# cptq/SignNet-BasisNet

Hardware: AMD Instinct MI355X
Metric: graphs/sec SignNet+GINE forward, ZINC batch=128 k=16 (higher is better)
Workload: dtype f32

## Files before the change

### signnet_basisnet_amd/csrc/fused_common.hpp

```cpp
#pragma once
#include "common.hpp"

namespace sn {

#ifdef SN_PROFILE
static __device__ long long g_prof[64];
#define SN_STAMP(i) do { if (sn_prof_on && blockIdx.x == 0 && threadIdx.x == 0) g_prof[i] = clock64(); } while (0)
#define SN_ACCUM(i, t0) do { if (sn_prof_on && blockIdx.x == 0 && threadIdx.x == 0) g_prof[i] += clock64() - (t0); } while (0)
#define SN_PROF_ON(cond) const bool sn_prof_on = (cond)
#else
#define SN_STAMP(i) do { } while (0)
#define SN_ACCUM(i, t0) do { } while (0)
#define SN_PROF_ON(cond) do { } while (0)
#endif

__device__ __forceinline__ f32x4 ld4(const float* __restrict__ p) {
  float4 t = *reinterpret_cast<const float4*>(p);
  return f32x4{t.x, t.y, t.z, t.w};
}
__device__ __forceinline__ f32x4 lds_ld4(const float* p) {
  float4 t = *reinterpret_cast<const float4*>(p);
  return f32x4{t.x, t.y, t.z, t.w};
}
__device__ __forceinline__ void lds_st4(float* p, f32x4 v) {
// ... 36 lines not shown
}
__device__ __forceinline__ Split8 split8(f32x4 a, f32x4 b) {
  const float x[8] = {a[0], a[1], a[2], a[3], b[0], b[1], b[2], b[3]};
  float h[8], m[8], l[8];
#pragma unroll
  for (int i = 0; i < 8; ++i) {
    h[i] = __uint_as_float(__float_as_uint(x[i]) & 0xffff0000u);
    const float r = x[i] - h[i];
    m[i] = __uint_as_float(__float_as_uint(r) & 0xffff0000u);
    l[i] = r - m[i];
  }
  Split8 s;
#pragma unroll
  for (int i = 0; i < 4; ++i) {
    s.h[i] = pack_hi16(h[2 * i], h[2 * i + 1]);
    s.m[i] = pack_hi16(m[2 * i], m[2 * i + 1]);
    s.l[i] = pack_hi16(l[2 * i], l[2 * i + 1]);
  }
  return s;
}
__device__ __forceinline__ void split4(f32x4 a, Split8& s, int half) {
  float h[4], m[4], l[4];
#pragma unroll
  for (int i = 0; i < 4; ++i) {
    h[i] = __uint_as_float(__float_as_uint(a[i]) & 0xffff0000u);
    const float r = a[i] - h[i];
    m[i] = __uint_as_float(__float_as_uint(r) & 0xffff0000u);
    l[i] = r - m[i];
  }
#pragma unroll
  for (int i = 0; i < 2; ++i) {
    s.h[2 * half + i] = pack_hi16(h[2 * i], h[2 * i + 1]);
    s.m[2 * half + i] = pack_hi16(m[2 * i], m[2 * i + 1]);
    s.l[2 * half + i] = pack_hi16(l[2 * i], l[2 * i + 1]);
  }
}
template <int NT>
__device__ __forceinline__ void split_rows(const f32x4 (&in)[NT], Split8 (&xs)[(NT + 1) / 2]) {
#pragma unroll
  for (int kb = 0; kb < (NT + 1) / 2; ++kb)
    xs[kb] = split8(in[2 * kb], (2 * kb + 1 < NT) ? in[2 * kb + 1] : f32x4{0.f, 0.f, 0.f, 0.f});
}
__device__ __forceinline__ f32x4 mfma_bf(u32x4 a, u32x4 b, f32x4 c) {
  return __builtin_amdgcn_mfma_f32_16x16x32_bf16(__builtin_bit_cast(bf16x8, a), __builtin_bit_cast(bf16x8, b), c, 0, 0, 0);
}
template <int N>
__device__ __forceinline__ void wait_vmcnt() { asm volatile("s_waitcnt vmcnt(%0)" ::"n"(N) : "memory"); }
__device__ __forceinline__ void lds_barrier() {
  asm volatile("s_waitcnt lgkmcnt(0)" ::: "memory");
  __builtin_amdgcn_s_barrier();
  asm volatile("" ::: "memory");
}

template <int NT, int NW = 4, int RING = SPLIT_RING>
struct WRing {
  static constexpr int NKB = (NT + 1) / 2;
  static constexpr int NF = 3 * NKB;
  static constexpr int NFE = NF + SPLIT_EPI;
  static constexpr int CHUNK = NFE * 1024;
  static constexpr int BYTES = RING * CHUNK;
  static constexpr int DEPTH = RING;
  static constexpr int LPC = (NFE + NW - 1) / NW;
  lds_char_t* base;
  int pos;
  int wave, lane;

  __device__ __forceinline__ void init(void* lds_base, int wave_, int lane_) {
    base = (lds_char_t*)lds_base; pos = 0; wave = wave_; lane = lane_;
  }
  template <int N>
  __device__ __forceinline__ void wait_shares() const { wait_vmcnt<N * LPC>(); }
  __device__ __forceinline__ int slot_of(int c) const {
    const int x = pos + c;
    if (RING == 3) return x - 3 * ((x * 43) >> 7);
    if (RING == 4) return x & 3;
    return x % RING;
  }
  __device__ __forceinline__ void issue(const void* w, int c, int slot) const {
    const __amdgpu_buffer_rsrc_t rs = weight_rsrc(reinterpret_cast<const float*>(w), 0x7fffffff);
    int wo = wave * 1024;
    asm volatile("" : "+s"(wo));
    lds_char_t* dst = base + slot * CHUNK + wo;
    const int src = c * CHUNK + wo;
#pragma unroll
    for (int f = 0; f < LPC; ++f) {
      int fo = NW * 1024 * f;
      if (NW * f + NW - 1 >= NFE) {
        const int last = (NFE - 1) * 1024 - wo;
        fo = fo < last ? fo : last;
      }
      __builtin_amdgcn_raw_ptr_buffer_load_lds(rs, (lds_void_t*)(dst + fo), 16, lane * 16, src + fo, 0, 0);
    }
  }
  __device__ __forceinline__ void prologue(const void* w, int nchunks) {
    lds_barrier();
    pos = 0;
#pragma unroll
    for (int c = 0; c < RING; ++c)
      if (c < nchunks) issue(w, c, c);
    if (nchunks >= RING) wait_shares<RING - 1>(); else wait_vmcnt<0>();
    lds_barrier();
  }
  __device__ __forceinline__ void drain() const { wait_vmcnt<0>(); }
};

struct WFrag { u32x4 h, m, l; };

template <int PREC>
__device__ __forceinline__ WFrag read_wfrag(const lds_char_t* p) {
  typedef __attribute__((address_space(3))) const u32x4 lds_u32x4;
  WFrag f;
  f.h = *(lds_u32x4*)(p);
  if constexpr (PREC <= PREC_HIGH) f.m = *(lds_u32x4*)(p + 1024); else f.m = u32x4{0u, 0u, 0u, 0u};
  if constexpr (PREC == PREC_HIGHEST) f.l = *(lds_u32x4*)(p + 2048); else f.l = u32x4{0u, 0u, 0u, 0u};
  return f;
}
template <int PREC, bool SWAP>
__device__ __forceinline__ void mm_reduced(const WFrag& f, const Split8& x, int kb, f32x4& a0, f32x4& a1) {
  static_assert(PREC == PREC_HIGH || PREC == PREC_MEDIUM, "the six-product form is written out at its call sites");
  if constexpr (PREC == PREC_HIGH) {
    a1 = SWAP ? mfma_bf(x.h, f.m, a1) : mfma_bf(f.m, x.h, a1);
    a0 = SWAP ? mfma_bf(x.m, f.h, a0) : mfma_bf(f.h, x.m, a0);
    a0 = SWAP ? mfma_bf(x.h, f.h, a0) : mfma_bf(f.h, x.h, a0);
  } else {
    f32x4& a = (kb & 1) ? a1 : a0;
    a = SWAP ? mfma_bf(x.h, f.h, a) : mfma_bf(f.h, x.h, a);
  }
}

template <int NT, int NTO, bool SWAP, bool EPIV = true, int NW = 4, int RING = SPLIT_RING, int PREC = PREC_HIGHEST, typename Pre, typename Epi>
__device__ __forceinline__ void wg_gemm_split(WRing<NT, NW, RING>& ring, const void* w, const void* wnext, bool live,
                                              const Split8 (&xs)[(NT + 1) / 2], Pre pre, Epi epi) {
  using R = WRing<NT, NW, RING>;
  constexpr int NKB = R::NKB;
  constexpr bool CHAIN = NTO >= RING;
  if (!CHAIN) ring.prologue(w, NTO);
  typedef __attribute__((address_space(3))) const f32x4 lds_f32x4;
  int sl[RING];
#pragma unroll
  for (int i = 0; i < RING; ++i) sl[i] = ring.slot_of(i);
  auto slot = [&](int c) { return sl[c % RING]; };
  auto stage = [&](int ot) {
    if (CHAIN) {
      const int pc = ot + RING;
      if (pc < NTO) ring.issue(w, pc, slot(ot)); else ring.issue(wnext, pc - NTO, slot(ot));
    }
  };
  if (live) {
    int ln16 = ring.lane * 16;
    asm volatile("" : "+v"(ln16));
    const lds_char_t* lbase = ring.base + ln16;
    auto rd = [&](int c, int kb) { return read_wfrag<PREC>(lbase + slot(c) * R::CHUNK + kb * 3072); };
    auto mm = [&](const WFrag& f, const Split8& x, int kb, f32x4& a0, f32x4& a1) {
      if constexpr (PREC != PREC_HIGHEST) {
        mm_reduced<PREC, SWAP>(f, x, kb, a0, a1);
      } else if (!SWAP) {
        a1 = mfma_bf(f.l, x.h, a1);
        a0 = mfma_bf(f.m, x.h, a0);
        a1 = mfma_bf(f.h, x.l, a1);
        a0 = mfma_bf(f.h, x.m, a0);
        a1 = mfma_bf(f.m, x.m, a1);
        a0 = mfma_bf(f.h, x.h, a0);
      } else {
        a1 = mfma_bf(x.h, f.l, a1);
        a0 = mfma_bf(x.h, f.m, a0);
        a1 = mfma_bf(x.l, f.h, a1);
        a0 = mfma_bf(x.m, f.h, a0);
        a1 = mfma_bf(x.m, f.m, a1);
        a0 = mfma_bf(x.h, f.h, a0);
      }
    };
    WFrag fa = rd(0, 0), fb;
#pragma unroll
    for (int ot = 0; ot < NTO; ++ot) {
      f32x4 a0 = {0.f, 0.f, 0.f, 0.f}, a1 = {0.f, 0.f, 0.f, 0.f};
      f32x4 e0 = {0.f, 0.f, 0.f, 0.f}, e1 = e0, e2 = e0;
      if (EPIV) {
        const lds_char_t* pe = lbase + slot(ot) * R::CHUNK + R::NF * 1024;
        e0 = *(lds_f32x4*)(pe); e1 = *(lds_f32x4*)(pe + 1024); e2 = *(lds_f32x4*)(pe + 2048);
      }
      const f32x4 pv = pre(ot);
#pragma unroll
      for (int kb = 0; kb + 1 < NKB; ++kb) {
        fb = rd(ot, kb + 1);
        __builtin_amdgcn_sched_barrier(0);
        mm(fa, xs[kb], kb, a0, a1);
        __builtin_amdgcn_sched_barrier(0);
        fa = fb;
      }
      if (CHAIN) {
        asm volatile("s_waitcnt lgkmcnt(0)" ::: "memory");
        ring.template wait_shares<RING - 2>();
        __builtin_amdgcn_s_barrier();
        asm volatile("" ::: "memory");
        stage(ot);
      }
      if (ot + 1 < NTO) fb = rd(ot + 1, 0);
      __builtin_amdgcn_sched_barrier(0);
      mm(fa, xs[NKB - 1], NKB - 1, a0, a1);
      __builtin_amdgcn_sched_barrier(0);
      epi(ot, a0 + a1, e0, e1, e2, pv);
      fa = fb;
    }
  } else if (CHAIN) {
#pragma unroll
    for (int ot = 0; ot < NTO; ++ot) {
      ring.template wait_shares<RING - 2>();
      __builtin_amdgcn_s_barrier();
      asm volatile("" ::: "memory");
      stage(ot);
    }
  }
  ring.pos = ring.slot_of(NTO);
}

constexpr int LAG_RING = 4;

template <int NT, int NW>
__device__ __forceinline__ void ring_prologue3(WRing<NT, NW, LAG_RING>& ring, const void* w) {
  lds_barrier();
  ring.pos = 0;
  ring.issue(w, 0, 0);
  ring.issue(w, 1, 1);
  ring.issue(w, 2, 2);
  ring.template wait_shares<2>();
  lds_barrier();
}

template <int NT, int NW>
__device__ __forceinline__ void ring_prologue3_issue(WRing<NT, NW, LAG_RING>& ring, const void* w) {
  lds_barrier();
  ring.pos = 0;
  ring.issue(w, 0, 0);
  ring.issue(w, 1, 1);
  ring.issue(w, 2, 2);
}

template <int NT, int NTO, int BAR_KB, int NW, int PREC = PREC_HIGHEST, typename Pre, typename Epi>
__device__ __forceinline__ void wg_gemm_split_lag(WRing<NT, NW, LAG_RING>& ring, const void* w, const void* wnext, bool live,
                                                  const Split8 (&xs)[(NT + 1) / 2], Pre pre, Epi epi) {
  using R = WRing<NT, NW, LAG_RING>;
  constexpr int NKB = R::NKB;
  static_assert(NTO >= 3 && BAR_KB >= 0 && BAR_KB < NKB, "look-ahead of three chunks; the barrier sits in front of a K block of the tile");
  typedef __attribute__((address_space(3))) const f32x4 lds_f32x4;
  int sl[LAG_RING];
#pragma unroll
  for (int i = 0; i < LAG_RING; ++i) sl[i] = ring.slot_of(i);
  auto slot = [&](int c) { return sl[c % LAG_RING]; };
  auto sync_stage = [&](int ot) {
    ring.template wait_shares<1>();
    __builtin_amdgcn_s_barrier();
    asm volatile("" ::: "memory");
    const int pc = ot + 3;
    if (pc < NTO) ring.issue(w, pc, slot(pc)); else ring.issue(wnext, pc - NTO, slot(pc));
  };
  if (live) {
    int ln16 = ring.lane * 16;
    asm volatile("" : "+v"(ln16));
    const lds_char_t* lbase = ring.base + ln16;
    auto rd = [&](int c, int kb) { return read_wfrag<PREC>(lbase + slot(c) * R::CHUNK + kb * 3072); };
    WFrag fa = rd(0, 0), fb;
#pragma unroll
    for (int ot = 0; ot < NTO; ++ot) {
      f32x4 a0 = {0.f, 0.f, 0.f, 0.f}, a1 = {0.f, 0.f, 0.f, 0.f};
      const lds_char_t* pe = lbase + slot(ot) * R::CHUNK + R::NF * 1024;
      const f32x4 e0 = *(lds_f32x4*)(pe), e1 = *(lds_f32x4*)(pe + 1024), e2 = *(lds_f32x4*)(pe + 2048);
      const f32x4 pv = pre(ot);
#pragma unroll
      for (int kb = 0; kb < NKB; ++kb) {
        if (kb == BAR_KB) sync_stage(ot);
        if (kb + 1 < NKB) fb = rd(ot, kb + 1);
        else if (ot + 1 < NTO) fb = rd(ot + 1, 0);
        __builtin_amdgcn_sched_barrier(0);
        if constexpr (PREC != PREC_HIGHEST) {
          mm_reduced<PREC, false>(fa, xs[kb], kb, a0, a1);
        } else {
          a1 = mfma_bf(fa.l, xs[kb].h, a1);
          a0 = mfma_bf(fa.m, xs[kb].h, a0);
          a1 = mfma_bf(fa.h, xs[kb].l, a1);
          a0 = mfma_bf(fa.h, xs[kb].m, a0);
          a1 = mfma_bf(fa.m, xs[kb].m, a1);
          a0 = mfma_bf(fa.h, xs[kb].h, a0);
        }
        __builtin_amdgcn_sched_barrier(0);
        fa = fb;
      }
      epi(ot, a0 + a1, e0, e1, e2, pv);
    }
  } else {
#pragma unroll
    for (int ot = 0; ot < NTO; ++ot) sync_stage(ot);
  }
  ring.pos = ring.slot_of(NTO);
}

__device__ __forceinline__ float row_allsum(float v) {
  v += __shfl_xor(v, 16, 64);
  v += __shfl_xor(v, 32, 64);
  return v;
}

struct NoPre { __device__ __forceinline__ f32x4 operator()(int) const { return f32x4{0.f, 0.f, 0.f, 0.f}; } };

}
```

### signnet_basisnet_amd/csrc/fused_rho.hip

```cpp
#include "fused_common.hpp"

namespace sn {

constexpr int RHO_R = SN_RHO_BIN_ROWS;

struct RhoStruct {
  const float* x;
  const float* eigvals;
  const int32_t* graph_ptr;
  const int32_t* rho_bin0;
  const int32_t* meta;
  int B;
  int kmax;
  int K;
  float* out_sum;
  const int32_t* node_graph;
  int N;
  const int32_t* bin_mem;
};

template <int NT, bool HP = false>
__device__ __forceinline__ void masked_layernorm(f32x4 (&v)[NT], const float* gamma , const float* beta ,
                                                 float eps, int d, int g, bool valid) {
  float s = 0.f;
#pragma unroll
  for (int kk = 0; kk < NT; ++kk) s += (v[kk][0] + v[kk][1]) + (v[kk][2] + v[kk][3]);
  const float mean = row_allsum(s) / (float)d;
  const bool last_ok = 16 * (NT - 1) + 4 * g < d;
  float q = 0.f;
#pragma unroll
  for (int kk = 0; kk < NT; ++kk) {
#pragma unroll
    for (int t = 0; t < 4; ++t) {
      const bool real = HP ? (16 * kk + 4 * g < d) : (kk + 1 < NT || last_ok);
      const float dlt = real ? v[kk][t] - mean : 0.f;
      q += dlt * dlt;
    }
  }
  const float rstd = 1.0f / sqrtf(row_allsum(q) / (float)d + eps);
#pragma unroll
  for (int kk = 0; kk < NT; ++kk) {
    const int c = 16 * kk + 4 * g;
    const f32x4 ga = lds_ld4(gamma + c), be = lds_ld4(beta + c);
    f32x4 o;
#pragma unroll
    for (int t = 0; t < 4; ++t) o[t] = valid ? (v[kk][t] - mean) * rstd * ga[t] + be[t] : 0.f;
    v[kk] = o;
  }
}

__device__ __forceinline__ float group_allmax(float v) {
  v = fmaxf(v, __shfl_xor(v, 16, 64));
  return fmaxf(v, __shfl_xor(v, 32, 64));
}
__device__ __forceinline__ float dpp_add(float v, int ctrl_sel) {
  const int x = __float_as_int(v);
  int y;
  switch (ctrl_sel) {
    case 0: y = __builtin_amdgcn_update_dpp(0, x, 0xB1, 0xf, 0xf, true); break;
    case 1: y = __builtin_amdgcn_update_dpp(0, x, 0x4E, 0xf, 0xf, true); break;
    case 2: y = __builtin_amdgcn_update_dpp(0, x, 0x141, 0xf, 0xf, true); break;
    default: y = __builtin_amdgcn_update_dpp(0, x, 0x140, 0xf, 0xf, true); break;
  }
  return v + __int_as_float(y);
}
__device__ __forceinline__ float tile_rowsum(float v) {
  v = dpp_add(v, 0);
  v = dpp_add(v, 1);
  v = dpp_add(v, 2);
  return dpp_add(v, 3);
}

template <int NT, bool REGATTN, bool ONE, bool HP = false, int NW = 4, int PREC = PREC_HIGHEST, bool RES3 = false>
__global__ __launch_bounds__(64 * NW, REGATTN ? (RES3 ? 3 : 2) : 1) void k_rho_fused(RhoStruct S, sn_rho_params P) {
  static_assert(NW == 4 || (NW == 8 && REGATTN), "eight waves: the register-attention variants only (no 64-row LDS images)");
  static_assert(!RES3 || (REGATTN && ONE && NW == 4), "three resident workgroups: the one-layer register-attention form only");
  constexpr int NTHR = 64 * NW;
  constexpr int D = 16 * NT;
  constexpr int LD = D + 4;
  constexpr int DKMAX = (D + 3) / 4;
  constexpr int NKB = (NT + 1) / 2;
  using Ring = WRing<NT, NW>;
  extern __shared__ __align__(1024) unsigned char lds_raw[];
  float* A = reinterpret_cast<float*>(lds_raw + Ring::BYTES);
  float* Bm = A + RHO_R * LD;
  __shared__ int s_graph;
  const int lane = threadIdx.x & 63, wave = __builtin_amdgcn_readfirstlane(threadIdx.x >> 6);
  const int r = wave * 16 + (lane & 15), g = lane >> 4, li = lane & 15;
  const int nbins = REGATTN ? (S.N + NW - 1) / NW : S.meta[4];
  const int d = P.d, H = P.heads, dk = d / H;
  f32x4 x[NT];
  int pf_gs = 0, pf_n = 0;
  auto fetch_rows = [&](int node_) {
    int slot_ = lane & 15, g_ = g;
    asm volatile("" : "+v"(slot_), "+v"(g_));
    const bool ok = node_ < S.N && slot_ < S.K;
    const float* xr = S.x + (ok ? ((int64_t)node_ * S.K + slot_) : (int64_t)0) * d;
#pragma unroll
    for (int kk = 0; kk < NT; ++kk) {
      const int c = 16 * kk + 4 * g_;
      const bool inb = HP ? c < d : (kk + 1 < NT || c < d);
      x[kk] = ld4(xr + (inb ? c : 0));
    }
  };
  auto fetch_graph = [&](int node_) {
    const int32_t* p = S.node_graph + (node_ < S.N ? node_ : 0);
    int gi;
    asm volatile("s_load_dword %0, %1, 0x0\n\ts_waitcnt lgkmcnt(0)" : "=s"(gi) : "s"(p) : "memory");
    const int32_t* q = S.graph_ptr + gi;
    long long rng;
    asm volatile("s_load_dwordx2 %0, %1, 0x0\n\ts_waitcnt lgkmcnt(0)" : "=s"(rng) : "s"(q) : "memory");
    pf_gs = (int)(rng & 0xffffffffll);
    pf_n = (int)(rng >> 32) - pf_gs;
  };
#ifdef SN_RHO_OLDSTART
  constexpr bool EARLY = false;
#else
  constexpr bool EARLY = REGATTN && (ONE || NT < 8);
#endif
  const int err = S.meta[5];
  const float temp = sqrtf((float)dk);
  const float rtemp = 1.0f / temp;
  { SN_PROF_ON(true); SN_STAMP(13); }
  float* lnv = reinterpret_cast<float*>(lds_raw + Ring::BYTES) + (REGATTN ? 0 : 2 * RHO_R * LD);
  Ring ring;
  ring.init(lds_raw, wave, lane);
  const void* wfirst = P.n_layers > 0 ? P.layers[0].wq : nullptr;
  const bool stream = NT >= SPLIT_RING && wfirst != nullptr && nbins > (int)blockIdx.x;
  if constexpr (EARLY && ONE && NT >= SPLIT_RING) {
    if (nbins <= (int)blockIdx.x) return;
    const int node0 = __builtin_amdgcn_readfirstlane((int)blockIdx.x * NW + wave);
    fetch_rows(node0);
    static_assert(4 * (D / 4) <= NTHR, "one float4 per thread covers the four vectors");
    const int li4 = (int)threadIdx.x < 4 * (D / 4) ? (int)threadIdx.x : 0;
    const sn_rho_layer& L0 = P.layers[0];
    const float *p0 = L0.ln1_g, *p1 = L0.ln1_b, *p2 = L0.ln2_g, *p3 = L0.ln2_b;
    asm volatile("" : "+s"(p0), "+s"(p1), "+s"(p2), "+s"(p3));
    const int lv = li4 / (D / 4), lc = 4 * (li4 - lv * (D / 4));
    typedef __attribute__((address_space(1))) const float gfloat_t;
    gfloat_t* src = (gfloat_t*)(lv == 0 ? p0 : (lv == 1 ? p1 : (lv == 2 ? p2 : p3)));
    const f32x4 lnr = f32x4{src[lc], src[lc + 1], src[lc + 2], src[lc + 3]};
    ring.pos = 0;
#pragma unroll
    for (int c = 0; c < Ring::DEPTH; ++c) ring.issue(wfirst, c, c);
    fetch_graph(node0);
    {
      typedef __attribute__((address_space(3))) float lds_float_t;
      const unsigned la = (unsigned)(size_t)(lds_float_t*)(lnv + 4 * li4);
      asm volatile("ds_write_b128 %0, %1" :: "v"(la), "v"(lnr) : "memory");
    }
    ring.template wait_shares<Ring::DEPTH - 1>();
    lds_barrier();
    if (err != 0) { ring.drain(); return; }
  } else {
    if constexpr (EARLY) {
      if (nbins > (int)blockIdx.x) {
        const int node0 = __builtin_amdgcn_readfirstlane((int)blockIdx.x * NW + wave);
        fetch_rows(node0);
        fetch_graph(node0);
      }
    } else {
      if (err != 0) return;
    }
    for (int i = threadIdx.x; i < P.n_layers * 4 * D; i += NTHR) {
      const int l = i / (4 * D), v = (i / D) & 3, c = i % D;
      const sn_rho_layer& Lq = P.layers[l];
      const float* src = v == 0 ? Lq.ln1_g : (v == 1 ? Lq.ln1_b : (v == 2 ? Lq.ln2_g : Lq.ln2_b));
      lnv[i] = src[c];
    }
    __syncthreads();
    if (stream) ring.prologue(wfirst, NT);
    if constexpr (EARLY) {
      if (err != 0) { ring.drain(); return; }
    }
  }

  for (int bin = blockIdx.x; bin < nbins; bin += gridDim.x) {
    SN_PROF_ON(bin == (int)blockIdx.x);
    SN_STAMP(0);
    int gs, n, kg, q, slot, node, kv, u0;
    bool unit_ok;
    if constexpr (REGATTN) {
      q = wave;
      slot = lane & 15;
      node = __builtin_amdgcn_readfirstlane(bin * NW + wave);
      unit_ok = node < S.N;
      if constexpr (EARLY) {
        gs = pf_gs;
        n = pf_n;
      } else {
        const int gi = unit_ok ? S.node_graph[node] : 0;
        gs = S.graph_ptr[gi];
        n = S.graph_ptr[gi + 1] - gs;
      }
      kg = (S.kmax > 0 && n > S.kmax) ? S.kmax : n;
      kv = unit_ok ? kg : 0;
      u0 = q * 16;
    } else {
      __syncthreads();
      for (int gq = threadIdx.x; gq < S.B; gq += NTHR)
        if (S.rho_bin0[gq] <= bin && bin < S.rho_bin0[gq + 1]) s_graph = gq;
      __syncthreads();
      const int gi = s_graph;
      gs = S.graph_ptr[gi];
      n = S.graph_ptr[gi + 1] - gs;
      kg = (S.kmax > 0 && n > S.kmax) ? S.kmax : n;
      const int pad = ((kg + 15) >> 4) << 4;
      const int upb = RHO_R / pad;
      q = r / pad;
      slot = r - q * pad;
      const int u = (bin - S.rho_bin0[gi]) * upb + q;
      unit_ok = q < upb && u < n;
      node = gs + u;
      kv = unit_ok ? kg : 0;
      u0 = q * pad;
    }
    const bool valid = unit_ok && slot < kg;
    constexpr bool mfma_attn = REGATTN;
    const bool wave_live = RES3 || __ballot(valid) != 0ull;
    float* Ar = A + r * LD;
    float* Br = Bm + r * LD;
// ... 144 lines not shown
            const float pj = expf(s - m);
            z += pj;
#pragma unroll
            for (int c = 0; c < DKMAX; c += 4)
              if (c < dk) { const f32x4 v4 = lds_ld4(vr + c); oh[c] += pj * v4[0]; oh[c + 1] += pj * v4[1]; oh[c + 2] += pj * v4[2]; oh[c + 3] += pj * v4[3]; }
          }
        } else {
          for (int j = 0; j < kv; ++j) {
            const float* kr = Bm + (u0 + j) * LD + hc;
            float s = 0.f;
#pragma unroll
            for (int c = 0; c < DKMAX; ++c)
              if (c < dk) s += qh[c] * kr[c];
            m = fmaxf(m, s);
          }
          for (int j = 0; j < kv; ++j) {
            const float* kr = Bm + (u0 + j) * LD + hc;
            const float* vr = A + (u0 + j) * LD + hc;
            float s = 0.f;
#pragma unroll
            for (int c = 0; c < DKMAX; ++c)
              if (c < dk) s += qh[c] * kr[c];
            const float pj = expf(s - m);
            z += pj;
#pragma unroll
            for (int c = 0; c < DKMAX; ++c)
              if (c < dk) oh[c] += pj * vr[c];
          }
        }
        const float zi = (kv > 0) ? 1.0f / z : 0.f;
        lds_barrier();
#pragma unroll
        for (int c = 0; c < DKMAX; ++c)
          if (c < dk) Br[hc + c] = oh[c] * zi;
        if (H * dk < D) {
          for (int c = H * dk + g; c < D; c += 4) Br[c] = 0.f;
        }
#pragma unroll
        for (int kk = 0; kk < NT; ++kk) o[kk] = lds_ld4(Br + 16 * kk + 4 * g);
        }
      }
      SN_STAMP(5);
      if (wave_live) split_rows<NT>(o, sp);
      if (ONE) load_x();
      wg_gemm_split<NT, NT, false, false, NW, SPLIT_RING, PREC>(ring, Lp.wfc, Lp.w1, wave_live, sp, NoPre(), [&](int ot, f32x4 acc, f32x4, f32x4, f32x4, f32x4) { x[ot] = acc + x[ot]; });
      SN_STAMP(6);
      if (wave_live) {
        int gl = g;
        asm volatile("" : "+v"(gl));
        masked_layernorm<NT, HP>(x, lnv + (l * 4 + 0) * D, lnv + (l * 4 + 1) * D, P.ln_eps, d, gl, valid);
        split_rows<NT>(x, sp);
      }
      SN_STAMP(7);
      wg_gemm_split<NT, NT, false, true, NW, SPLIT_RING, PREC>(ring, Lp.w1, Lp.w2, wave_live, sp, NoPre(), [&](int ot, f32x4 acc, f32x4 b1, f32x4, f32x4, f32x4) { o[ot] = relu4(acc + b1); });
      SN_STAMP(8);
      if (wave_live) split_rows<NT>(o, sp);
#ifdef SN_PROFILE
      asm volatile("" :: "v"(sp[0].h), "v"(last_plane<PREC>(sp[NKB - 1])));
#endif
      SN_STAMP(14);
      wg_gemm_split<NT, NT, false, true, NW, SPLIT_RING, PREC>(ring, Lp.w2, wafter, wave_live, sp, NoPre(), [&](int ot, f32x4 acc, f32x4 b2, f32x4, f32x4, f32x4) { x[ot] = acc + b2 + x[ot]; });
      SN_STAMP(9);
      if (wave_live) {
        int gl = g;
        asm volatile("" : "+v"(gl));
        masked_layernorm<NT, HP>(x, lnv + (l * 4 + 2) * D, lnv + (l * 4 + 3) * D, P.ln_eps, d, gl, valid);
      }
      SN_STAMP(10);
    }
    if (mfma_attn) {
      if (wave_live) {
        float* orow = S.out_sum + (int64_t)node * d;
        int g_ = g;
        asm volatile("" : "+v"(g_));
#pragma unroll
        for (int kk = 0; kk < NT; ++kk) {
          f32x4 s;
#pragma unroll
          for (int t = 0; t < 4; ++t) s[t] = tile_rowsum(valid ? x[kk][t] : 0.f);
          const int c = 16 * kk + 4 * g_;
          if (li == 0 && unit_ok && (HP ? c < d : (kk + 1 < NT || c < d))) *reinterpret_cast<float4*>(orow + c) = make_float4(s[0], s[1], s[2], s[3]);
        }
      }
      if (EARLY && bin + (int)gridDim.x < nbins) {
        const int nnode = __builtin_amdgcn_readfirstlane((bin + (int)gridDim.x) * NW + wave);
        fetch_rows(nnode);
        fetch_graph(nnode);
      }
    } else {
#pragma unroll
      for (int kk = 0; kk < NT; ++kk) lds_st4(Br + 16 * kk + 4 * g, valid ? x[kk] : f32x4{0.f, 0.f, 0.f, 0.f});
      __syncthreads();
      if (valid && slot == 0) {
        float* orow = S.out_sum + (int64_t)node * d;
#pragma unroll
        for (int kk = 0; kk < NT; ++kk) {
          const int c = 16 * kk + 4 * g;
          f32x4 s = {0.f, 0.f, 0.f, 0.f};
          for (int j = 0; j < kv; ++j) s += lds_ld4(Bm + (u0 + j) * LD + c);
          if (kk + 1 < NT || c < d) *reinterpret_cast<float4*>(orow + c) = make_float4(s[0], s[1], s[2], s[3]);
        }
      }
    }
  }
  { SN_PROF_ON(true); SN_STAMP(11); }
  ring.drain();
}

template <int NT, bool ONE, bool COLS, int PREC = PREC_HIGHEST>
__global__ __launch_bounds__(RHO_R * 4, ONE ? 2 : 1) void k_rho_wide(RhoStruct S, sn_rho_params P) {
  static_assert(NT == 4 || NT == 8, "head width 16 or 32");
  constexpr int D = 16 * NT;
  constexpr int LD = D + 4;
  constexpr int NKB = (NT + 1) / 2;
  constexpr int CPH = NT / 4;
  using Ring = WRing<NT>;
  extern __shared__ __align__(1024) unsigned char lds_raw[];
  float* IMG = reinterpret_cast<float*>(lds_raw + Ring::BYTES);
  float* lnv = IMG + RHO_R * LD;
  const int lane = threadIdx.x & 63, wave = __builtin_amdgcn_readfirstlane(threadIdx.x >> 6);
  const int r = wave * 16 + (lane & 15), g = lane >> 4, li = lane & 15;
  const int nb_raw = COLS ? S.meta[7] : S.meta[4];
  const int m_err = S.meta[5] | (COLS ? S.meta[1] : 0);
  const int nbins = m_err != 0 ? 0 : nb_raw;
  const int d = P.d;
  const float rtemp = 1.0f / sqrtf((float)(d / P.heads));
  Ring ring;
  ring.init(lds_raw, wave, lane);
  const void* wfirst = P.n_layers > 0 ? P.layers[0].wq : nullptr;
  if constexpr (ONE) {
    static_assert(4 * (D / 4) <= RHO_R * 4, "one float4 per thread covers the four vectors");
    const int li4 = (int)threadIdx.x < 4 * (D / 4) ? (int)threadIdx.x : 0;
    const sn_rho_layer& L0 = P.layers[0];
    const float *p0 = L0.ln1_g, *p1 = L0.ln1_b, *p2 = L0.ln2_g, *p3 = L0.ln2_b;
    asm volatile("" : "+s"(p0), "+s"(p1), "+s"(p2), "+s"(p3));
    const int lv = li4 / (D / 4), lc = 4 * (li4 - lv * (D / 4));
    typedef __attribute__((address_space(1))) const float gfloat_t;
    gfloat_t* src = (gfloat_t*)(lv == 0 ? p0 : (lv == 1 ? p1 : (lv == 2 ? p2 : p3)));
    const f32x4 lnr = f32x4{src[lc], src[lc + 1], src[lc + 2], src[lc + 3]};
    if (nbins <= (int)blockIdx.x) return;
    ring.pos = 0;
#pragma unroll
    for (int c = 0; c < Ring::DEPTH; ++c) ring.issue(wfirst, c, c);
    {
      typedef __attribute__((address_space(3))) float lds_float_t;
      const unsigned la = (unsigned)(size_t)(lds_float_t*)(lnv + 4 * li4);
      asm volatile("ds_write_b128 %0, %1" :: "v"(la), "v"(lnr) : "memory");
    }
    ring.template wait_shares<Ring::DEPTH - 1>();
    lds_barrier();
  } else {
    for (int i = threadIdx.x; i < P.n_layers * 4 * D; i += RHO_R * 4) {
      const int l = i / (4 * D), v = (i / D) & 3, c = i % D;
      const sn_rho_layer& Lq = P.layers[l];
      const float* src = v == 0 ? Lq.ln1_g : (v == 1 ? Lq.ln1_b : (v == 2 ? Lq.ln2_g : Lq.ln2_b));
      lnv[i] = src[c];
    }
    __syncthreads();
    if (wfirst != nullptr && nbins > (int)blockIdx.x) ring.prologue(wfirst, NT);
  }
  float* IMGr = IMG + r * LD;

  for (int bin = blockIdx.x; bin < nbins; bin += gridDim.x) {
    int m_off[8], m_len[8], m_node[8], m_gs[8];
    if constexpr (COLS) {
      typedef int i32x16 __attribute__((ext_vector_type(16)));
      i32x16 rw;
      {
        const int32_t* rec = S.bin_mem + (int64_t)bin * 16;
        asm volatile("s_load_dwordx16 %0, %1, 0x0\n\ts_waitcnt lgkmcnt(0)" : "=s"(rw) : "s"(rec) : "memory");
      }
#pragma unroll
      for (int k = 0; k < 8; ++k) {
        const int w0 = rw[2 * k], g0 = rw[2 * k + 1];
        const int n = ((w0 >> 25) & 63) + 1;
        m_off[k] = (w0 >> 19) & 63;
        m_len[k] = (w0 >= 0 && n <= S.K) ? n : 0;
        m_node[k] = g0 + ((w0 >> 13) & 63);
        m_gs[k] = g0;
      }
    } else {
      int lo = 0, hi = S.B;
      while (hi - lo > 1) {
        const int mid = (lo + hi) >> 1;
        if (S.rho_bin0[mid] <= bin) lo = mid; else hi = mid;
      }
      const int gs = S.graph_ptr[lo], n = S.graph_ptr[lo + 1] - gs;
      const int kg = (S.kmax > 0 && n > S.kmax) ? S.kmax : n;
      const int pad = ((kg + 15) >> 4) << 4;
      const int upb = RHO_R / pad;
      const int ub = (bin - S.rho_bin0[lo]) * upb;
#pragma unroll
      for (int k = 0; k < 8; ++k) {
        m_off[k] = k * pad;
        m_len[k] = (k < upb && ub + k < n) ? kg : 0;
        m_node[k] = gs + ub + k;
        m_gs[k] = gs;
      }
    }
    int u0 = 0, kv = 0, node = 0, gsr = 0;
    int klo = RHO_R, khi = 0;
#pragma unroll
    for (int k = 0; k < 8; ++k) {
      if (r >= m_off[k] && r < m_off[k] + m_len[k]) { u0 = m_off[k]; kv = m_len[k]; node = m_node[k]; gsr = m_gs[k]; }
      if (m_len[k] > 0 && m_off[k] < wave * 16 + 16 && m_off[k] + m_len[k] > wave * 16) {
        klo = min(klo, m_off[k]);
        khi = max(khi, m_off[k] + m_len[k]);
      }
    }
// ... 58 lines not shown
#pragma unroll
          for (int h = 0; h < 4; ++h) {
            float m = -INFINITY;
#pragma unroll
            for (int kt = 0; kt < 4; ++kt)
#pragma unroll
              for (int t = 0; t < 4; ++t)
                if ((unsigned)(16 * kt + 4 * g + t - u0) < (unsigned)kv) m = fmaxf(m, sc[h][kt][t]);
            m = group_allmax(m);
            float z = 0.f;
#pragma unroll
            for (int kt = 0; kt < 4; ++kt)
#pragma unroll
              for (int t = 0; t < 4; ++t) {
                const float e = ((unsigned)(16 * kt + 4 * g + t - u0) < (unsigned)kv) ? expf(sc[h][kt][t] - m) : 0.f;
                sc[h][kt][t] = e;
                z += e;
              }
            z = row_allsum(z);
            const float zi = (kv > 0 && z > 0.f) ? 1.0f / z : 0.f;
#pragma unroll
            for (int kt = 0; kt < 4; ++kt)
#pragma unroll
              for (int t = 0; t < 4; ++t) sc[h][kt][t] *= zi;
          }
        }
        lds_barrier();
        wg_gemm_split<NT, NT, false, false, 4, SPLIT_RING, PREC>(ring, Lp.wv, Lp.wfc, wave_live, sp, NoPre(), [&](int ot, f32x4 acc, f32x4, f32x4, f32x4, f32x4) { lds_st4(IMGr + 16 * ot + 4 * g, acc); });
        lds_barrier();
#pragma unroll
        for (int ot = 0; ot < NT; ++ot) {
          f32x4 acc = {0.f, 0.f, 0.f, 0.f};
#pragma unroll
          for (int kt = 0; kt < 4; ++kt)
            if (wave_live && kt >= kt_lo && kt < kt_hi) {
              const float* vr = IMG + (16 * kt + 4 * g) * LD + 16 * ot + li;
              acc = mfma16(vr[0], sc[ot / CPH][kt][0], acc);
              acc = mfma16(vr[LD], sc[ot / CPH][kt][1], acc);
              acc = mfma16(vr[2 * LD], sc[ot / CPH][kt][2], acc);
              acc = mfma16(vr[3 * LD], sc[ot / CPH][kt][3], acc);
            }
          o[ot] = acc;
        }
      }
      if (wave_live) split_rows<NT>(o, sp);
      if (ONE) load_x();
      wg_gemm_split<NT, NT, false, false, 4, SPLIT_RING, PREC>(ring, Lp.wfc, Lp.w1, wave_live, sp, NoPre(), [&](int ot, f32x4 acc, f32x4, f32x4, f32x4, f32x4) { x[ot] = acc + x[ot]; });
      if (wave_live) {
        int gl = g;
        asm volatile("" : "+v"(gl));
        masked_layernorm<NT>(x, lnv + (l * 4 + 0) * D, lnv + (l * 4 + 1) * D, P.ln_eps, d, gl, valid);
        split_rows<NT>(x, sp);
      }
      wg_gemm_split<NT, NT, false, true, 4, SPLIT_RING, PREC>(ring, Lp.w1, Lp.w2, wave_live, sp, NoPre(), [&](int ot, f32x4 acc, f32x4 b1, f32x4, f32x4, f32x4) { o[ot] = relu4(acc + b1); });
      if (wave_live) split_rows<NT>(o, sp);
      wg_gemm_split<NT, NT, false, true, 4, SPLIT_RING, PREC>(ring, Lp.w2, wafter, wave_live, sp, NoPre(), [&](int ot, f32x4 acc, f32x4 b2, f32x4, f32x4, f32x4) { x[ot] = acc + b2 + x[ot]; });
      if (wave_live) {
        int gl = g;
        asm volatile("" : "+v"(gl));
        masked_layernorm<NT>(x, lnv + (l * 4 + 2) * D, lnv + (l * 4 + 3) * D, P.ln_eps, d, gl, valid);
      }
    }
#pragma unroll
    for (int kk = 0; kk < NT; ++kk) lds_st4(IMGr + 16 * kk + 4 * g, valid ? x[kk] : f32x4{0.f, 0.f, 0.f, 0.f});
    lds_barrier();
    {
      int mo = 0, ml = 0;
#pragma unroll
      for (int k = 0; k < 8; ++k)
        if (li == k) { mo = m_off[k]; ml = m_len[k]; }
      int nd[4];
      bool st[4];
#pragma unroll
      for (int t = 0; t < 4; ++t) {
        nd[t] = g == 0 ? m_node[t] : m_node[4 + t];
        st[t] = g < 2 && (g == 0 ? m_len[t] : m_len[4 + t]) > 0;
      }
#pragma unroll
      for (int j = 0; j < CPH; ++j) {
        const int ct = wave * CPH + j;
        const float* xc = IMG + g * LD + 16 * ct + li;
        f32x4 acc = {0.f, 0.f, 0.f, 0.f};
#pragma unroll
        for (int s = 0; s < RHO_R / 4; ++s) {
          const float a = ((unsigned)(4 * s + g - mo) < (unsigned)ml) ? 1.f : 0.f;
          acc = mfma16(a, xc[4 * s * LD], acc);
        }
#pragma unroll
        for (int t = 0; t < 4; ++t)
          if (st[t]) S.out_sum[(int64_t)nd[t] * D + 16 * ct + li] = acc[t];
      }
    }
  }
  ring.drain();
}

template <int NT, bool ONE, bool COLS, int PREC = PREC_HIGHEST>
static int launch_rho_wide(const RhoStruct& S, const sn_rho_params& P, int64_t bins_bound, hipStream_t st) {
  constexpr int LD = 16 * NT + 4;
  const size_t lds_fixed = (size_t)WRing<NT>::BYTES + (size_t)(RHO_R * LD) * sizeof(float);
  const size_t lds_max = lds_fixed + (size_t)SN_RHO_MAX_LAYERS * 4 * 16 * NT * sizeof(float);
  const size_t lds = lds_fixed + (size_t)(P.n_layers > 0 ? P.n_layers : 1) * 4 * 16 * NT * sizeof(float);
  static int cus = 0;
  if (cus == 0) {
    if (lds_max > 64 * 1024 &&
        hipFuncSetAttribute(reinterpret_cast<const void*>(k_rho_wide<NT, ONE, COLS, PREC>), hipFuncAttributeMaxDynamicSharedMemorySize,
                            (int)lds_max) != hipSuccess)
      return fail(SN_ERR_LAUNCH, "sn_rho_fused_f32: cannot raise the dynamic LDS limit to %zu", lds_max);
    int dev = 0, n = 256;
    if (hipGetDevice(&dev) == hipSuccess) hipDeviceGetAttribute(&n, hipDeviceAttributeMultiprocessorCount, dev);
    cus = n > 0 ? n : 256;
  }
  int64_t grid = bins_bound < (int64_t)2 * cus ? bins_bound : (int64_t)2 * cus;
  if (grid < 1) grid = 1;
  hipLaunchKernelGGL((k_rho_wide<NT, ONE, COLS, PREC>), dim3((unsigned)grid), dim3(RHO_R * 4), lds, st, S, P);
  return SN_OK;
}

static bool rho_three_resident() {
  static int v = -1;
  if (v < 0) { const char* e = getenv("SN_RHO_RESIDENT"); v = (e && e[0] == '2') ? 0 : 1; }
  return v == 1;
}

template <int NT, bool REGATTN, bool ONE, bool HP = false, int NW = 4, int PREC = PREC_HIGHEST, bool RES3 = false>
static int launch_rho(const RhoStruct& S, const sn_rho_params& P, int64_t bins_bound, hipStream_t st) {
  constexpr int LD = 16 * NT + 4;
  const size_t lds_fixed = (size_t)WRing<NT, NW>::BYTES + (REGATTN ? 0 : (size_t)(2 * RHO_R * LD) * sizeof(float));
  const size_t lds_max = lds_fixed + (size_t)SN_RHO_MAX_LAYERS * 4 * 16 * NT * sizeof(float);
  const size_t lds = lds_fixed + (size_t)(P.n_layers > 0 ? P.n_layers : 1) * 4 * 16 * NT * sizeof(float);
  static int cus = 0;
  if (cus == 0) {
    if (lds_max > 64 * 1024 &&
        hipFuncSetAttribute(reinterpret_cast<const void*>(k_rho_fused<NT, REGATTN, ONE, HP, NW, PREC, RES3>), hipFuncAttributeMaxDynamicSharedMemorySize,
                            (int)lds_max) != hipSuccess)
      return fail(SN_ERR_LAUNCH, "sn_rho_fused_f32: cannot raise the dynamic LDS limit to %zu", lds_max);
    int dev = 0, n = 256;
    if (hipGetDevice(&dev) == hipSuccess) hipDeviceGetAttribute(&n, hipDeviceAttributeMultiprocessorCount, dev);
    cus = n > 0 ? n : 256;
  }
  constexpr bool three = REGATTN && ONE && NW == 4 && (RES3 || (NT == 4 && PREC == PREC_HIGHEST));
  const int64_t bins = REGATTN ? ((int64_t)S.N + NW - 1) / NW : bins_bound;
  const int64_t per_cu = NW == 8 ? 1 : ((three && rho_three_resident() && bins > (int64_t)2 * cus) ? 3 : 2);
  int64_t grid = bins_bound < per_cu * cus ? bins_bound : per_cu * cus;
#ifdef SN_RHO_GRID1
  grid = cus;
#endif
  if (grid < 1) grid = 1;
  hipLaunchKernelGGL((k_rho_fused<NT, REGATTN, ONE, HP, NW, PREC, RES3>), dim3((unsigned)grid), dim3(64 * NW), lds, st, S, P);
  return SN_OK;
}

static bool rho_eight_waves() {
  static int v = -1;
  if (v < 0) { const char* e = getenv("SN_RHO_WAVES"); v = (e && e[0] == '8') ? 1 : 0; }
  return v == 1;
}

template <bool REGATTN, bool ONE, int PREC = PREC_HIGHEST>
static int dispatch_rho(int nt, const RhoStruct& S, const sn_rho_params& P, int64_t bound, hipStream_t st) {
  if constexpr (PREC != PREC_HIGHEST) {
    switch (nt) {
      case 4: return launch_rho<4, REGATTN, ONE, false, 4, PREC>(S, P, bound, st);
      case 7: return launch_rho<7, REGATTN, ONE, false, 4, PREC>(S, P, bound, st);
      case 8: return launch_rho<8, REGATTN, ONE, false, 4, PREC>(S, P, bound, st);
    }
    return fail(SN_ERR_UNSUPPORTED, "sn_rho_fused_prec_f32: matmul precision %d is built for hidden widths with ceil(d/16) in {4, 7, 8} "
                "(got d = %d); SN_PREC_HIGHEST serves every width", PREC, P.d);
  } else {
    if constexpr (REGATTN) {
      if (rho_eight_waves()) {
        if (nt == 8) return launch_rho<8, true, ONE, false, 8>(S, P, bound, st);
        if (nt == 4) return launch_rho<4, true, ONE, false, 8>(S, P, bound, st);
      }
    }
    if constexpr (REGATTN && ONE) {
      if (nt == 8 && rho_three_resident()) return launch_rho<8, true, true, false, 4, PREC_HIGHEST, true>(S, P, bound, st);
    }
    switch (nt) {
      case 1: return launch_rho<1, REGATTN, ONE>(S, P, bound, st);
      case 2: return launch_rho<2, REGATTN, ONE>(S, P, bound, st);
      case 3: return launch_rho<3, REGATTN, ONE>(S, P, bound, st);
      case 4: return launch_rho<4, REGATTN, ONE>(S, P, bound, st);
// ... 105 lines not shown
```

Measured before the change: 552,000.

## Keep rho MLP biases resident in LDS instead of streaming them per chunk

The weight ring for the rho kernels no longer streams each chunk's epilogue (bias) vectors alongside the split weights. Instead, the w1/w2 biases of every layer are loaded once into the LDS layer-vector table, next to the layernorm parameters, and the GEMM epilogue reads them from there. This shrinks every ring slot and the number of buffer loads issued per weight chunk, which lowers LDS footprint and global traffic in the streamed MLP. In exchange the per-layer LDS table grows from four to six vectors, and the setup gathers bias words from the packed weight layout.

```diff
diff --git a/signnet_basisnet_amd/csrc/fused_common.hpp b/signnet_basisnet_amd/csrc/fused_common.hpp
--- a/signnet_basisnet_amd/csrc/fused_common.hpp
+++ b/signnet_basisnet_amd/csrc/fused_common.hpp
@@ -112,15 +112,17 @@
   asm volatile("" ::: "memory");
 }
 
-template <int NT, int NW = 4, int RING = SPLIT_RING>
+template <int NT, int NW = 4, int RING = SPLIT_RING, bool EF = true>
 struct WRing {
   static constexpr int NKB = (NT + 1) / 2;
   static constexpr int NF = 3 * NKB;
   static constexpr int NFE = NF + SPLIT_EPI;
   static constexpr int CHUNK = NFE * 1024;
-  static constexpr int BYTES = RING * CHUNK;
+  static constexpr int NST = EF ? NFE : NF;
+  static constexpr int SLOT = NST * 1024;
+  static constexpr int BYTES = RING * SLOT;
   static constexpr int DEPTH = RING;
-  static constexpr int LPC = (NFE + NW - 1) / NW;
+  static constexpr int LPC = (NST + NW - 1) / NW;
   lds_char_t* base;
   int pos;
   int wave, lane;
@@ -140,13 +142,13 @@
     const __amdgpu_buffer_rsrc_t rs = weight_rsrc(reinterpret_cast<const float*>(w), 0x7fffffff);
     int wo = wave * 1024;
     asm volatile("" : "+s"(wo));
-    lds_char_t* dst = base + slot * CHUNK + wo;
+    lds_char_t* dst = base + slot * SLOT + wo;
     const int src = c * CHUNK + wo;
 #pragma unroll
     for (int f = 0; f < LPC; ++f) {
       int fo = NW * 1024 * f;
-      if (NW * f + NW - 1 >= NFE) {
-        const int last = (NFE - 1) * 1024 - wo;
+      if (NW * f + NW - 1 >= NST) {
+        const int last = (NST - 1) * 1024 - wo;
         fo = fo < last ? fo : last;
       }
       __builtin_amdgcn_raw_ptr_buffer_load_lds(rs, (lds_void_t*)(dst + fo), 16, lane * 16, src + fo, 0, 0);
@@ -188,10 +190,10 @@
   }
 }
 
-template <int NT, int NTO, bool SWAP, bool EPIV = true, int NW = 4, int RING = SPLIT_RING, int PREC = PREC_HIGHEST, typename Pre, typename Epi>
-__device__ __forceinline__ void wg_gemm_split(WRing<NT, NW, RING>& ring, const void* w, const void* wnext, bool live,
-                                              const Split8 (&xs)[(NT + 1) / 2], Pre pre, Epi epi) {
-  using R = WRing<NT, NW, RING>;
+template <int NT, int NTO, bool SWAP, bool EPIV = true, int NW = 4, int RING = SPLIT_RING, int PREC = PREC_HIGHEST, bool EF = true, typename Pre, typename Epi>
+__device__ __forceinline__ void wg_gemm_split(WRing<NT, NW, RING, EF>& ring, const void* w, const void* wnext, bool live,
+                                              const Split8 (&xs)[(NT + 1) / 2], Pre pre, Epi epi, int etab = 0) {
+  using R = WRing<NT, NW, RING, EF>;
   constexpr int NKB = R::NKB;
   constexpr bool CHAIN = NTO >= RING;
   if (!CHAIN) ring.prologue(w, NTO);
@@ -210,7 +212,11 @@
     int ln16 = ring.lane * 16;
     asm volatile("" : "+v"(ln16));
     const lds_char_t* lbase = ring.base + ln16;
-    auto rd = [&](int c, int kb) { return read_wfrag<PREC>(lbase + slot(c) * R::CHUNK + kb * 3072); };
+    auto rd = [&](int c, int kb) { return read_wfrag<PREC>(lbase + slot(c) * R::SLOT + kb * 3072); };
+    int eo = 0;
+    if constexpr (EPIV && !EF) {
+      eo = etab + ((ln16 >> 8) << 4);
+    }
     auto mm = [&](const WFrag& f, const Split8& x, int kb, f32x4& a0, f32x4& a1) {
       if constexpr (PREC != PREC_HIGHEST) {
         mm_reduced<PREC, SWAP>(f, x, kb, a0, a1);
@@ -235,9 +241,12 @@
     for (int ot = 0; ot < NTO; ++ot) {
       f32x4 a0 = {0.f, 0.f, 0.f, 0.f}, a1 = {0.f, 0.f, 0.f, 0.f};
       f32x4 e0 = {0.f, 0.f, 0.f, 0.f}, e1 = e0, e2 = e0;
-      if (EPIV) {
-        const lds_char_t* pe = lbase + slot(ot) * R::CHUNK + R::NF * 1024;
+      if constexpr (EPIV && EF) {
+        const lds_char_t* pe = lbase + slot(ot) * R::SLOT + R::NF * 1024;
         e0 = *(lds_f32x4*)(pe); e1 = *(lds_f32x4*)(pe + 1024); e2 = *(lds_f32x4*)(pe + 2048);
+      } else if constexpr (EPIV) {
+        const lds_char_t* pe = ring.base + eo + 64 * ot;
+        e0 = *(lds_f32x4*)(pe); e1 = *(lds_f32x4*)(pe + 64 * NT); e2 = *(lds_f32x4*)(pe + 128 * NT);
       }
       const f32x4 pv = pre(ot);
 #pragma unroll
@@ -296,10 +305,10 @@
   ring.issue(w, 2, 2);
 }
 
-template <int NT, int NTO, int BAR_KB, int NW, int PREC = PREC_HIGHEST, typename Pre, typename Epi>
-__device__ __forceinline__ void wg_gemm_split_lag(WRing<NT, NW, LAG_RING>& ring, const void* w, const void* wnext, bool live,
-                                                  const Split8 (&xs)[(NT + 1) / 2], Pre pre, Epi epi) {
-  using R = WRing<NT, NW, LAG_RING>;
+template <int NT, int NTO, int BAR_KB, int NW, int PREC = PREC_HIGHEST, bool EF = true, typename Pre, typename Epi>
+__device__ __forceinline__ void wg_gemm_split_lag(WRing<NT, NW, LAG_RING, EF>& ring, const void* w, const void* wnext, bool live,
+                                                  const Split8 (&xs)[(NT + 1) / 2], Pre pre, Epi epi, int etab = 0) {
+  using R = WRing<NT, NW, LAG_RING, EF>;
   constexpr int NKB = R::NKB;
   static_assert(NTO >= 3 && BAR_KB >= 0 && BAR_KB < NKB, "look-ahead of three chunks; the barrier sits in front of a K block of the tile");
   typedef __attribute__((address_space(3))) const f32x4 lds_f32x4;
@@ -318,13 +327,18 @@
     int ln16 = ring.lane * 16;
     asm volatile("" : "+v"(ln16));
     const lds_char_t* lbase = ring.base + ln16;
-    auto rd = [&](int c, int kb) { return read_wfrag<PREC>(lbase + slot(c) * R::CHUNK + kb * 3072); };
+    auto rd = [&](int c, int kb) { return read_wfrag<PREC>(lbase + slot(c) * R::SLOT + kb * 3072); };
+    int eo = 0;
+    if constexpr (!EF) {
+      eo = etab + ((ln16 >> 8) << 4);
+    }
     WFrag fa = rd(0, 0), fb;
 #pragma unroll
     for (int ot = 0; ot < NTO; ++ot) {
       f32x4 a0 = {0.f, 0.f, 0.f, 0.f}, a1 = {0.f, 0.f, 0.f, 0.f};
-      const lds_char_t* pe = lbase + slot(ot) * R::CHUNK + R::NF * 1024;
-      const f32x4 e0 = *(lds_f32x4*)(pe), e1 = *(lds_f32x4*)(pe + 1024), e2 = *(lds_f32x4*)(pe + 2048);
+      const lds_char_t* pe = EF ? lbase + slot(ot) * R::SLOT + R::NF * 1024 : ring.base + eo + 64 * ot;
+      constexpr int ES = EF ? 1024 : 64 * NT;
+      const f32x4 e0 = *(lds_f32x4*)(pe), e1 = *(lds_f32x4*)(pe + ES), e2 = *(lds_f32x4*)(pe + 2 * ES);
       const f32x4 pv = pre(ot);
 #pragma unroll
       for (int kb = 0; kb < NKB; ++kb) {
diff --git a/signnet_basisnet_amd/csrc/fused_rho.hip b/signnet_basisnet_amd/csrc/fused_rho.hip
--- a/signnet_basisnet_amd/csrc/fused_rho.hip
+++ b/signnet_basisnet_amd/csrc/fused_rho.hip
@@ -3,6 +3,14 @@
 namespace sn {
 
 constexpr int RHO_R = SN_RHO_BIN_ROWS;
+
+template <int NT, int NW = 4>
+using RhoRing = WRing<NT, NW, SPLIT_RING, false>;
+constexpr int RHO_LAYER_VECS = 6;
+template <typename R>
+__device__ __forceinline__ constexpr int rho_bias_word(int c) {
+  return ((c >> 4) * R::CHUNK + R::NF * 1024 + ((c >> 2) & 3) * 256) / 4 + (c & 3);
+}
 
 struct RhoStruct {
   const float* x;
@@ -80,7 +88,7 @@
   constexpr int LD = D + 4;
   constexpr int DKMAX = (D + 3) / 4;
   constexpr int NKB = (NT + 1) / 2;
-  using Ring = WRing<NT, NW>;
+  using Ring = RhoRing<NT, NW>;
   extern __shared__ __align__(1024) unsigned char lds_raw[];
   float* A = reinterpret_cast<float*>(lds_raw + Ring::BYTES);
   float* Bm = A + RHO_R * LD;
@@ -122,7 +130,10 @@
   const float temp = sqrtf((float)dk);
   const float rtemp = 1.0f / temp;
   { SN_PROF_ON(true); SN_STAMP(13); }
-  float* lnv = reinterpret_cast<float*>(lds_raw + Ring::BYTES) + (REGATTN ? 0 : 2 * RHO_R * LD);
+  constexpr int LNV_OFF = Ring::BYTES + (REGATTN ? 0 : 2 * RHO_R * LD * (int)sizeof(float));
+  float* lnv = reinterpret_cast<float*>(lds_raw + LNV_OFF);
+  const int n_lay = ONE ? 1 : P.n_layers;
+  auto bias_off = [&](int l, int v) { return LNV_OFF + ((n_lay * 4 + l * 2 + v) * D) * (int)sizeof(float); };
   Ring ring;
   ring.init(lds_raw, wave, lane);
   const void* wfirst = P.n_layers > 0 ? P.layers[0].wq : nullptr;
@@ -131,14 +142,16 @@
     if (nbins <= (int)blockIdx.x) return;
     const int node0 = __builtin_amdgcn_readfirstlane((int)blockIdx.x * NW + wave);
     fetch_rows(node0);
-    static_assert(4 * (D / 4) <= NTHR, "one float4 per thread covers the four vectors");
-    const int li4 = (int)threadIdx.x < 4 * (D / 4) ? (int)threadIdx.x : 0;
+    static_assert(6 * (D / 4) <= NTHR, "one float4 per thread covers the six vectors");
+    const int li4 = (int)threadIdx.x < 6 * (D / 4) ? (int)threadIdx.x : 0;
     const sn_rho_layer& L0 = P.layers[0];
     const float *p0 = L0.ln1_g, *p1 = L0.ln1_b, *p2 = L0.ln2_g, *p3 = L0.ln2_b;
-    asm volatile("" : "+s"(p0), "+s"(p1), "+s"(p2), "+s"(p3));
-    const int lv = li4 / (D / 4), lc = 4 * (li4 - lv * (D / 4));
+    const float *p4 = reinterpret_cast<const float*>(L0.w1), *p5 = reinterpret_cast<const float*>(L0.w2);
+    asm volatile("" : "+s"(p0), "+s"(p1), "+s"(p2), "+s"(p3), "+s"(p4), "+s"(p5));
+    const int lv = li4 / (D / 4), lq = li4 - lv * (D / 4);
+    const int lc = lv < 4 ? 4 * lq : rho_bias_word<Ring>(4 * lq);
     typedef __attribute__((address_space(1))) const float gfloat_t;
-    gfloat_t* src = (gfloat_t*)(lv == 0 ? p0 : (lv == 1 ? p1 : (lv == 2 ? p2 : p3)));
+    gfloat_t* src = (gfloat_t*)(lv == 0 ? p0 : (lv == 1 ? p1 : (lv == 2 ? p2 : (lv == 3 ? p3 : (lv == 4 ? p4 : p5)))));
     const f32x4 lnr = f32x4{src[lc], src[lc + 1], src[lc + 2], src[lc + 3]};
     ring.pos = 0;
 #pragma unroll
@@ -167,6 +180,10 @@
       const sn_rho_layer& Lq = P.layers[l];
       const float* src = v == 0 ? Lq.ln1_g : (v == 1 ? Lq.ln1_b : (v == 2 ? Lq.ln2_g : Lq.ln2_b));
       lnv[i] = src[c];
+    }
+    for (int i = threadIdx.x; i < P.n_layers * 2 * D; i += NTHR) {
+      const sn_rho_layer& Lq = P.layers[i / (2 * D)];
+      lnv[P.n_layers * 4 * D + i] = reinterpret_cast<const float*>((i / D) & 1 ? Lq.w2 : Lq.w1)[rho_bias_word<Ring>(i % D)];
     }
     __syncthreads();
     if (stream) ring.prologue(wfirst, NT);
@@ -417,14 +434,14 @@
         split_rows<NT>(x, sp);
       }
       SN_STAMP(7);
-      wg_gemm_split<NT, NT, false, true, NW, SPLIT_RING, PREC>(ring, Lp.w1, Lp.w2, wave_live, sp, NoPre(), [&](int ot, f32x4 acc, f32x4 b1, f32x4, f32x4, f32x4) { o[ot] = relu4(acc + b1); });
+      wg_gemm_split<NT, NT, false, true, NW, SPLIT_RING, PREC>(ring, Lp.w1, Lp.w2, wave_live, sp, NoPre(), [&](int ot, f32x4 acc, f32x4 b1, f32x4, f32x4, f32x4) { o[ot] = relu4(acc + b1); }, bias_off(l, 0));
       SN_STAMP(8);
       if (wave_live) split_rows<NT>(o, sp);
 #ifdef SN_PROFILE
       asm volatile("" :: "v"(sp[0].h), "v"(last_plane<PREC>(sp[NKB - 1])));
 #endif
       SN_STAMP(14);
-      wg_gemm_split<NT, NT, false, true, NW, SPLIT_RING, PREC>(ring, Lp.w2, wafter, wave_live, sp, NoPre(), [&](int ot, f32x4 acc, f32x4 b2, f32x4, f32x4, f32x4) { x[ot] = acc + b2 + x[ot]; });
+      wg_gemm_split<NT, NT, false, true, NW, SPLIT_RING, PREC>(ring, Lp.w2, wafter, wave_live, sp, NoPre(), [&](int ot, f32x4 acc, f32x4 b2, f32x4, f32x4, f32x4) { x[ot] = acc + b2 + x[ot]; }, bias_off(l, 1));
       SN_STAMP(9);
       if (wave_live) {
         int gl = g;
@@ -479,10 +496,13 @@
   constexpr int LD = D + 4;
   constexpr int NKB = (NT + 1) / 2;
   constexpr int CPH = NT / 4;
-  using Ring = WRing<NT>;
+  using Ring = RhoRing<NT>;
   extern __shared__ __align__(1024) unsigned char lds_raw[];
   float* IMG = reinterpret_cast<float*>(lds_raw + Ring::BYTES);
+  constexpr int LNV_OFF = Ring::BYTES + RHO_R * LD * (int)sizeof(float);
   float* lnv = IMG + RHO_R * LD;
+  const int n_lay = ONE ? 1 : P.n_layers;
+  auto bias_off = [&](int l, int v) { return LNV_OFF + ((n_lay * 4 + l * 2 + v) * D) * (int)sizeof(float); };
   const int lane = threadIdx.x & 63, wave = __builtin_amdgcn_readfirstlane(threadIdx.x >> 6);
   const int r = wave * 16 + (lane & 15), g = lane >> 4, li = lane & 15;
   const int nb_raw = COLS ? S.meta[7] : S.meta[4];
@@ -494,14 +514,16 @@
   ring.init(lds_raw, wave, lane);
   const void* wfirst = P.n_layers > 0 ? P.layers[0].wq : nullptr;
   if constexpr (ONE) {
-    static_assert(4 * (D / 4) <= RHO_R * 4, "one float4 per thread covers the four vectors");
-    const int li4 = (int)threadIdx.x < 4 * (D / 4) ? (int)threadIdx.x : 0;
+    static_assert(6 * (D / 4) <= RHO_R * 4, "one float4 per thread covers the six vectors");
+    const int li4 = (int)threadIdx.x < 6 * (D / 4) ? (int)threadIdx.x : 0;
     const sn_rho_layer& L0 = P.layers[0];
     const float *p0 = L0.ln1_g, *p1 = L0.ln1_b, *p2 = L0.ln2_g, *p3 = L0.ln2_b;
-    asm volatile("" : "+s"(p0), "+s"(p1), "+s"(p2), "+s"(p3));
-    const int lv = li4 / (D / 4), lc = 4 * (li4 - lv * (D / 4));
+    const float *p4 = reinterpret_cast<const float*>(L0.w1), *p5 = reinterpret_cast<const float*>(L0.w2);
+    asm volatile("" : "+s"(p0), "+s"(p1), "+s"(p2), "+s"(p3), "+s"(p4), "+s"(p5));
+    const int lv = li4 / (D / 4), lq = li4 - lv * (D / 4);
+    const int lc = lv < 4 ? 4 * lq : rho_bias_word<Ring>(4 * lq);
     typedef __attribute__((address_space(1))) const float gfloat_t;
-    gfloat_t* src = (gfloat_t*)(lv == 0 ? p0 : (lv == 1 ? p1 : (lv == 2 ? p2 : p3)));
+    gfloat_t* src = (gfloat_t*)(lv == 0 ? p0 : (lv == 1 ? p1 : (lv == 2 ? p2 : (lv == 3 ? p3 : (lv == 4 ? p4 : p5)))));
     const f32x4 lnr = f32x4{src[lc], src[lc + 1], src[lc + 2], src[lc + 3]};
     if (nbins <= (int)blockIdx.x) return;
     ring.pos = 0;
@@ -520,6 +542,10 @@
       const sn_rho_layer& Lq = P.layers[l];
       const float* src = v == 0 ? Lq.ln1_g : (v == 1 ? Lq.ln1_b : (v == 2 ? Lq.ln2_g : Lq.ln2_b));
       lnv[i] = src[c];
+    }
+    for (int i = threadIdx.x; i < P.n_layers * 2 * D; i += RHO_R * 4) {
+      const sn_rho_layer& Lq = P.layers[i / (2 * D)];
+      lnv[P.n_layers * 4 * D + i] = reinterpret_cast<const float*>((i / D) & 1 ? Lq.w2 : Lq.w1)[rho_bias_word<Ring>(i % D)];
     }
     __syncthreads();
     if (wfirst != nullptr && nbins > (int)blockIdx.x) ring.prologue(wfirst, NT);
@@ -684,9 +710,9 @@
         masked_layernorm<NT>(x, lnv + (l * 4 + 0) * D, lnv + (l * 4 + 1) * D, P.ln_eps, d, gl, valid);
         split_rows<NT>(x, sp);
       }
-      wg_gemm_split<NT, NT, false, true, 4, SPLIT_RING, PREC>(ring, Lp.w1, Lp.w2, wave_live, sp, NoPre(), [&](int ot, f32x4 acc, f32x4 b1, f32x4, f32x4, f32x4) { o[ot] = relu4(acc + b1); });
+      wg_gemm_split<NT, NT, false, true, 4, SPLIT_RING, PREC>(ring, Lp.w1, Lp.w2, wave_live, sp, NoPre(), [&](int ot, f32x4 acc, f32x4 b1, f32x4, f32x4, f32x4) { o[ot] = relu4(acc + b1); }, bias_off(l, 0));
       if (wave_live) split_rows<NT>(o, sp);
-      wg_gemm_split<NT, NT, false, true, 4, SPLIT_RING, PREC>(ring, Lp.w2, wafter, wave_live, sp, NoPre(), [&](int ot, f32x4 acc, f32x4 b2, f32x4, f32x4, f32x4) { x[ot] = acc + b2 + x[ot]; });
+      wg_gemm_split<NT, NT, false, true, 4, SPLIT_RING, PREC>(ring, Lp.w2, wafter, wave_live, sp, NoPre(), [&](int ot, f32x4 acc, f32x4 b2, f32x4, f32x4, f32x4) { x[ot] = acc + b2 + x[ot]; }, bias_off(l, 1));
       if (wave_live) {
         int gl = g;
         asm volatile("" : "+v"(gl));
@@ -730,9 +756,9 @@
 template <int NT, bool ONE, bool COLS, int PREC = PREC_HIGHEST>
 static int launch_rho_wide(const RhoStruct& S, const sn_rho_params& P, int64_t bins_bound, hipStream_t st) {
   constexpr int LD = 16 * NT + 4;
-  const size_t lds_fixed = (size_t)WRing<NT>::BYTES + (size_t)(RHO_R * LD) * sizeof(float);
-  const size_t lds_max = lds_fixed + (size_t)SN_RHO_MAX_LAYERS * 4 * 16 * NT * sizeof(float);
-  const size_t lds = lds_fixed + (size_t)(P.n_layers > 0 ? P.n_layers : 1) * 4 * 16 * NT * sizeof(float);
+  const size_t lds_fixed = (size_t)RhoRing<NT>::BYTES + (size_t)(RHO_R * LD) * sizeof(float);
+  const size_t lds_max = lds_fixed + (size_t)SN_RHO_MAX_LAYERS * RHO_LAYER_VECS * 16 * NT * sizeof(float);
+  const size_t lds = lds_fixed + (size_t)(P.n_layers > 0 ? P.n_layers : 1) * RHO_LAYER_VECS * 16 * NT * sizeof(float);
   static int cus = 0;
   if (cus == 0) {
     if (lds_max > 64 * 1024 &&
@@ -758,9 +784,9 @@
 template <int NT, bool REGATTN, bool ONE, bool HP = false, int NW = 4, int PREC = PREC_HIGHEST, bool RES3 = false>
 static int launch_rho(const RhoStruct& S, const sn_rho_params& P, int64_t bins_bound, hipStream_t st) {
   constexpr int LD = 16 * NT + 4;
-  const size_t lds_fixed = (size_t)WRing<NT, NW>::BYTES + (REGATTN ? 0 : (size_t)(2 * RHO_R * LD) * sizeof(float));
-  const size_t lds_max = lds_fixed + (size_t)SN_RHO_MAX_LAYERS * 4 * 16 * NT * sizeof(float);
-  const size_t lds = lds_fixed + (size_t)(P.n_layers > 0 ? P.n_layers : 1) * 4 * 16 * NT * sizeof(float);
+  const size_t lds_fixed = (size_t)RhoRing<NT, NW>::BYTES + (REGATTN ? 0 : (size_t)(2 * RHO_R * LD) * sizeof(float));
+  const size_t lds_max = lds_fixed + (size_t)SN_RHO_MAX_LAYERS * RHO_LAYER_VECS * 16 * NT * sizeof(float);
+  const size_t lds = lds_fixed + (size_t)(P.n_layers > 0 ? P.n_layers : 1) * RHO_LAYER_VECS * 16 * NT * sizeof(float);
   static int cus = 0;
   if (cus == 0) {
     if (lds_max > 64 * 1024 &&
```

Result: no change. 551,500 (-0.1%).
